# autonomousvision/unimatch

Measured on AMD Instinct MI355X. Metric: image_pairs_per_sec, higher is better.
Workload: dtype f16x2

## Files before the change

include/unimatch_hip.h:

```cpp
#ifndef UNIMATCH_HIP_H
#define UNIMATCH_HIP_H

#include <stddef.h>
#include <stdint.h>

#ifdef __cplusplus
extern "C" {
#endif

#define UM_VERSION 220

#define UM_MODE_EXACT 0
#define UM_MODE_FAST 1

#define UM_ERR_BAD_ARG (-1)
#define UM_ERR_BAD_GEOMETRY (-2)
#define UM_ERR_WORKSPACE (-3)
#define UM_ERR_UNSUPPORTED (-4)
#define UM_ERR_COLLECTIVE (-5)

int um_version(void);
const char* um_last_error_string(void);

#define UM_RANGE_PLANES 1u
// ... 21 lines not shown
#define UM_K_COUNT 12
#define UM_V_WATTN_TILE 0
#define UM_V_WATTN_KSPLIT 1
#define UM_V_FFN_TILE 2
#define UM_V_FFN_HSPLIT 3
#define UM_V_GSV4 4
#define UM_V_GSV3 5
#define UM_V_K4_MFMA 6
#define UM_V_K4_VALU 7
#define UM_V_K3_MFMA 8
#define UM_V_K3_VALU 9
#define UM_V_CONV_PATCH 10
#define UM_V_CONV_ROWS 11
#define UM_V_CONV_GENERIC 12
#define UM_V_WATTN_W8 13
#define UM_V_COUNT 14
int um_census_enable(int on);
long um_census_count(int variant);
int um_window_attn_tile_census(int enable, unsigned long long* counts4);
double um_probe_mfma_flops(int iters);
int um_probe_mfma(float* sink, int iters, void* stream);
int um_probe_copy(const void* src, void* dst, size_t bytes, void* stream);
int um_probe_chase(const unsigned* ring, unsigned* out, int hops, void* stream);
int um_timing_enable(int kernel_mask);
int um_timing_collect(int kernel_id, double* total_ms, int* launches);

size_t um_window_attn_workspace_bytes(int streams, int tokens, int channels, int mode);
int um_window_attn_fwd(const float* q, const float* k, const float* v, float* out,
                       int streams, int h, int w, int channels,
                       int win_h, int win_w, int shift_h, int shift_w,
                       int mode, void* workspace, size_t workspace_bytes, void* stream);
// ... 62 lines not shown

size_t um_stem_planes_bytes(int batch, int h, int w);
size_t um_conv7_planes_bytes(int batch, int h, int w, int stride);
int um_conv7_fwd(const float* image, int channels, int normalize, const float* mean3, const float* std3, void* image_planes,
                 const void* w_planes, const float* bias, float* out, int out_ld, int out_coff, void* out_planes, int outp_ld,
                 int outp_coff, long outp_rows, float* stats_out, int batch, int h, int w, int cout, int stride, int act,
                 int wshift, void* stream);
int um_stem_conv_fwd(const float* image, int normalize, const float* mean3, const float* std3, void* image_planes,
                     const void* w_planes, float* out, float* stats_out, int batch, int h, int w, int cout, int wshift,
                     void* stream);

size_t um_nhwc_norm_workspace_bytes(int batch, int pixels, int channels);
int um_nhwc_instance_norm(const float* x, const float* shortcut, const void* shortcut_planes, void* planes_out, float* f32_out,
                          int batch, int pixels, int channels, float eps, int normalize, int relu, const float* conv_stats,
                          int conv_stats_parts, void* workspace, size_t workspace_bytes, int mode, void* stream);

int um_nhwc_gate(int mode, const float* src, int src_ld, const float* zr, float* hbuf, void* planes_out, int ld, int coff,
                 long plane_rows, long rows, int channels, void* stream);

int um_nchw_to_nhwc(const float* x, void* planes_out, float* f32_out, int batch, int channels, int pixels, int mode,
                    void* stream);

size_t um_global_corr_workspace_bytes(int batch, int tokens, int channels, int mode);
int um_global_corr_softmax_flow(const float* f0, const float* f1, float* flow,
                                int batch, int h, int w, int channels, int bidir,
                                int mode, void* workspace, size_t workspace_bytes, void* stream);

int um_global_corr_softmax_stereo(const float* f0, const float* f1, float* disp,
                                  int batch, int h, int w, int channels,
                                  int mode, void* workspace, size_t workspace_bytes, void* stream);
// ... 96 lines not shown
```

unimatch_amd/_abi.py:

```python
import ctypes
import os

_HERE = os.path.dirname(os.path.abspath(__file__))
LIB_PATH = os.environ.get('UM_LIB') or os.path.join(_HERE, 'libunimatch_hip.so')

MODE_EXACT = 0
MODE_FAST = 1

CENSUS = {'wattn_tile': 0, 'wattn_ksplit': 1, 'ffn_tile': 2, 'ffn_hsplit': 3, 'gsv4': 4, 'gsv3': 5, 'k4_mfma': 6, 'k4_valu': 7,
          'k3_mfma': 8, 'k3_valu': 9, 'conv_patch': 10, 'conv_rows': 11, 'conv_generic': 12, 'wattn_w8': 13}

_c_int, _c_size_t, _c_void_p = ctypes.c_int, ctypes.c_size_t, ctypes.c_void_p

SIGNATURES = {
    'um_version': (_c_int, []),
    'um_last_error_string': (ctypes.c_char_p, []),
    'um_range_flags': (_c_int, [ctypes.POINTER(ctypes.c_uint), _c_int]),
    'um_timing_enable': (_c_int, [_c_int]),
    'um_timing_collect': (_c_int, [_c_int, ctypes.POINTER(ctypes.c_double), ctypes.POINTER(_c_int)]),
    'um_window_attn_workspace_bytes': (_c_size_t, [_c_int] * 4),
    'um_window_attn_fwd': (_c_int, [_c_void_p] * 4 + [_c_int] * 9 + [_c_void_p, _c_size_t, _c_void_p]),
    'um_window_attn_planes_fwd': (_c_int, [_c_void_p] * 4 + [_c_int] * 6 + [ctypes.c_long] * 2 + [_c_int] * 6 + [_c_void_p]),
    'um_window_attn_merge_fwd': (_c_int, [_c_void_p] * 7 + [ctypes.c_float, _c_int, _c_void_p] + [_c_int] * 6 + [ctypes.c_long] * 2 +
                                 [_c_int] * 6 + [_c_void_p]),
    'um_window_attn_qproj_merge_fwd': (_c_int, [_c_void_p] * 8 + [ctypes.c_float, _c_int, _c_void_p] + [_c_int] * 5 + [ctypes.c_long] +
# ... 9 lines not shown
                                _c_void_p]),
    'um_ffn_split_workspace_bytes': (_c_size_t, [_c_int] * 2),
    'um_ffn_kv_fwd': (_c_int, [_c_void_p] * 4 + [_c_int] * 3 + [_c_void_p] * 2 + [ctypes.c_float, _c_void_p, _c_void_p, _c_void_p, _c_int, _c_void_p,
                                _c_size_t, _c_void_p]),
    'um_kv4_fwd': (_c_int, [_c_void_p, _c_void_p, _c_int, _c_int, _c_void_p, _c_int, _c_void_p]),
    'um_conv2d_fwd': (_c_int, [_c_void_p] * 5 + [_c_int] * 13 + [_c_void_p]),
    'um_conv2d_ex': (_c_int, [_c_void_p, _c_int, _c_int, ctypes.c_long, _c_void_p, _c_void_p, _c_void_p, _c_int, _c_int, _c_void_p,
                              _c_int, _c_int, ctypes.c_long, _c_void_p] + [_c_int] * 13 + [_c_void_p]),
    'um_nhwc_gate': (_c_int, [_c_int, _c_void_p, _c_int, _c_void_p, _c_void_p, _c_void_p, _c_int, _c_int, ctypes.c_long, ctypes.c_long,
                              _c_int, _c_void_p]),
    'um_local_corr_with_flow_planes': (_c_int, [_c_void_p] * 4 + [_c_int, ctypes.c_long] + [_c_int] * 5 + [_c_void_p]),
    'um_conv2d_gru_fwd': (_c_int, [_c_int, _c_void_p, _c_int, _c_int, ctypes.c_long, _c_void_p, _c_void_p, _c_void_p, _c_void_p, _c_int,
                                   _c_void_p, _c_int, _c_void_p, _c_int, _c_int, ctypes.c_long] + [_c_int] * 11 + [_c_void_p]),
    'um_conv2d_gru_add_fwd': (_c_int, [_c_int, _c_void_p, _c_int, _c_int, ctypes.c_long, _c_void_p, _c_void_p, _c_void_p, _c_int, _c_void_p, _c_void_p,
                                        _c_int, _c_void_p, _c_int, _c_void_p, _c_int, _c_int, ctypes.c_long] + [_c_int] * 11 + [_c_void_p]),
    'um_conv_stats_bytes': (_c_size_t, [_c_int] * 3),
    'um_conv_stats_parts': (_c_int, [_c_int] * 8),
    'um_stem_planes_bytes': (_c_size_t, [_c_int] * 3),
    'um_conv7_planes_bytes': (_c_size_t, [_c_int] * 4),
    'um_conv7_fwd': (_c_int, [_c_void_p, _c_int, _c_int] + [_c_void_p] * 6 + [_c_int, _c_int, _c_void_p, _c_int, _c_int, ctypes.c_long,
                              _c_void_p] + [_c_int] * 7 + [_c_void_p]),
    'um_stem_conv_fwd': (_c_int, [_c_void_p, _c_int] + [_c_void_p] * 6 + [_c_int] * 5 + [_c_void_p]),
    'um_nhwc_norm_workspace_bytes': (_c_size_t, [_c_int] * 3),
    'um_nhwc_instance_norm': (_c_int, [_c_void_p] * 5 + [_c_int] * 3 + [ctypes.c_float, _c_int, _c_int, _c_void_p, _c_int, _c_void_p,
                                       _c_size_t, _c_int, _c_void_p]),
    'um_nchw_to_nhwc': (_c_int, [_c_void_p] * 3 + [_c_int] * 4 + [_c_void_p]),
    'um_flow_warp': (_c_int, [_c_void_p] * 3 + [_c_int] * 4 + [_c_void_p]),
    'um_fwd_bwd_occlusion': (_c_int, [_c_void_p] * 4 + [_c_int] * 3 + [ctypes.c_float] * 2 + [_c_void_p]),
    'um_flow_to_rgb_workspace_bytes': (_c_size_t, [_c_int] * 3),
    'um_flow_to_rgb': (_c_int, [_c_void_p] * 2 + [_c_int] * 3 + [_c_void_p, _c_size_t, _c_void_p]),
# ... 136 lines not shown
```

unimatch_amd/csrc/conv.hip:

```cpp
#include <cstdlib>
#include <cstring>
#ifndef UM_CONV_2P
#define UM_CONV_2P 0
#endif
#include "common.h"
#include "planes.h"

struct ConvArgs {
    const unsigned short* ap;
    long a_plane_stride;
    unsigned row_stride;
    unsigned zero_row;
    const unsigned short* wp;
    long w_plane_stride;
    const float* bias;
    float* out;
    unsigned short* outp;
    long outp_plane_stride;
    int out_ld, out_coff, outp_ld, outp_coff;
    int act;
    int gate, gate_c, gate_zld;
    float* gate_h;
    const float* gate_z;
    float* gate_hout;
    int gate_hout_ld;
    float* stats;
    const float* addend;
    int addend_ld;
    int B, Hi, Wi, Cin, Ho, Wo, Cout;
    int KH, KW, stride, pad_h, pad_w;
    int M;
    float out_scale;
    int xcd;
};

__device__ __forceinline__ void conv_dma16(const void* base, unsigned byte_off, const unsigned char* lds_dst) {
    const unsigned dst = __builtin_amdgcn_readfirstlane(
        (unsigned)(unsigned long)(const __attribute__((address_space(3))) unsigned char*)lds_dst);
    unsigned keep;
    asm volatile("s_mov_b32 %0, m0\n\ts_mov_b32 m0, %3\n\ts_nop 0\n\tglobal_load_lds_dwordx4 %1, %2\n\ts_mov_b32 m0, %0"
                 : "=&s"(keep)
                 : "v"(byte_off), "s"(base), "s"(dst)
                 : "memory");
}

template <int V>
struct IntC {
    static constexpr int value = V;
// ... 550 lines not shown
template <int NS, int NT>
struct ConvPatchLds {
    static constexpr int NTE = NT < 2 ? NT : 2;
    static constexpr int PW = 34, PPIX = 10 * PW;
    static constexpr int PROWS = 352;
    static constexpr int ATILE = PROWS * 32;
    static constexpr int WTILE = 32 * NT * 32;
    static constexpr int ASLOT = NS * ATILE, WSLOT = NS * 3 * WTILE;
    static constexpr int WBASE = 2 * ASLOT;
    static constexpr int STAGES = 2 * ASLOT + 2 * WSLOT;
    static constexpr int EPI = 8 * 32 * (32 * NTE * 4);
    static constexpr int SCRATCH = 8 * 2 * 32 * NT * 4 + 64;
    static constexpr int TOTAL = (STAGES > EPI + SCRATCH) ? STAGES : EPI + SCRATCH;
};

template <typename T, int NS, int NT>
__global__ __launch_bounds__(512, (NT < 4 ? 2 : 1)) void conv_patch_kernel(ConvArgs a) {
    using L = ConvPatchLds<NS, NT>;
    constexpr int ATILE = L::ATILE, WTILE = L::WTILE, ASLOT = L::ASLOT, WSLOT = L::WSLOT, WBASE = L::WBASE;
    constexpr int PW = L::PW;
    extern __shared__ __attribute__((aligned(16))) unsigned char lds[];

    const int tid = threadIdx.x, lane = tid & 63;
    const int wave = __builtin_amdgcn_readfirstlane(tid >> 6);
    const int half = lane >> 5, fr = lane & 31;
    const int twn = (a.Wo + 31) >> 5, tpi = twn * ((a.Ho + 7) >> 3);
    const int ny = (a.Cout + 32 * NT - 1) / (32 * NT);
    const int wg = a.xcd ? xcd_remap(blockIdx.x, gridDim.x) : blockIdx.x;
    const int tile = wg / ny;
    const int bt = tile / tpi, tt = tile - bt * tpi;
    const int ty = tt / twn, tx = tt - ty * twn;
    const int y0 = ty * 8, x0 = tx * 32;
    const int n0 = (wg - tile * ny) * (32 * NT);
    const int cpt = a.Cin >> 4;
    const int ktot = 9 * a.Cin;

    const int dcp = lane & 1;
    unsigned rowoff[2];
#pragma unroll
    for (int i = 0; i < 2; ++i) {
        const int j = 32 * (wave + 8 * i) + (lane >> 1);
        const int py = j / PW, px = j - py * PW;
        const int iy = y0 - 1 + py, ix = x0 - 1 + px;
        const bool ok = j < L::PPIX && (unsigned)iy < (unsigned)a.Hi && (unsigned)ix < (unsigned)a.Wi;
        const unsigned row = ok ? (unsigned)((bt * a.Hi + iy) * a.Wi + ix) : a.zero_row;
        rowoff[i] = row * a.row_stride;
    }
    auto stage_patch = [&](int cc, unsigned char* buf) {
#pragma unroll
        for (int i = 0; i < 2; ++i)
            if (i == 0 || wave < 3) {
                const int blk = wave + 8 * i;
                const int r = 32 * blk + (lane >> 1);
                const int sc = dcp ^ ((r >> 3) & 1);
                const unsigned off = rowoff[i] + (unsigned)((cc * 16 + 8 * sc) * 2);
#pragma unroll
                for (int pl = 0; pl < NS; ++pl) conv_dma16(a.ap + pl * a.a_plane_stride, off, buf + pl * ATILE + (32 * blk) * 32);
            }
    };
    auto stage_w = [&](int cc, int ky, unsigned char* buf) {
#pragma unroll
        for (int k = 0; k < (3 * NT + 7) / 8; ++k) {
            const int q = wave + 8 * k;
            if (q < 3 * NT) {
                const int kx = q / NT, jb = q - kx * NT;
                const int r = 32 * jb + (lane >> 1);
                const int sc = dcp ^ ((r >> 3) & 1);
                const int n = min(n0 + r, a.Cout - 1);
                const unsigned off = (unsigned)(((long)n * ktot + (ky * 3 + kx) * a.Cin + cc * 16 + 8 * sc) * 2);
#pragma unroll
                for (int pl = 0; pl < NS; ++pl)
                    conv_dma16(a.wp + pl * a.w_plane_stride, off, buf + (kx * NS + pl) * WTILE + (32 * jb) * 32);
            }
// ... 4 lines not shown
#pragma unroll
    for (int nt = 0; nt < NT; ++nt)
#pragma unroll
        for (int r = 0; r < 16; ++r) acc[nt][r] = 0.f;

    const int foffw = fr * 32 + ((half ^ ((fr >> 3) & 1)) << 4);
    int foffa[3][3];
#pragma unroll
    for (int ky = 0; ky < 3; ++ky)
#pragma unroll
        for (int kx = 0; kx < 3; ++kx) {
            const int r = (wave + ky) * PW + kx + fr;
            foffa[ky][kx] = r * 32 + ((half ^ ((r >> 3) & 1)) << 4);
        }

    stage_patch(0, lds);
    stage_w(0, 0, lds + WBASE);
    asm volatile("s_waitcnt vmcnt(0)" ::: "memory");
    __syncthreads();

    for (int cc = 0; cc < cpt; ++cc) {
        const int a_cur = (cc & 1) * ASLOT, a_nxt = ASLOT - a_cur;
#pragma unroll
        for (int ky = 0; ky < 3; ++ky) {
            const int w_par = (cc + ky) & 1;
            const int w_cur = WBASE + w_par * WSLOT, w_nxt = WBASE + (w_par ^ 1) * WSLOT;
            const bool last = ky == 2 && cc + 1 == cpt;
            __builtin_amdgcn_s_setprio(1);
#pragma unroll
            for (int kx = 0; kx < 3; ++kx) {
                if (kx == 0 && !last) stage_w(ky == 2 ? cc + 1 : cc, ky == 2 ? 0 : ky + 1, lds + w_nxt);
                if (kx == 1 && ky == 0 && cc + 1 < cpt) stage_patch(cc + 1, lds + a_nxt);
                const i16x8 bh = *reinterpret_cast<const i16x8*>(lds + a_cur + foffa[ky][kx]);
                i16x8 bl;
                if (NS == 2) bl = *reinterpret_cast<const i16x8*>(lds + a_cur + ATILE + foffa[ky][kx]);
                const unsigned char* wt = lds + w_cur + kx * NS * WTILE;
#pragma unroll
                for (int nt = 0; nt < NT; ++nt) {
                    const i16x8 wh = *reinterpret_cast<const i16x8*>(wt + nt * 32 * 32 + foffw);
                    if (NS == 2) {
                        const i16x8 wl = *reinterpret_cast<const i16x8*>(wt + WTILE + nt * 32 * 32 + foffw);
                        if (UM_CONV_2P != 1) acc[nt] = T::mfma(wl, bh, acc[nt]);
                        if (UM_CONV_2P != 2) acc[nt] = T::mfma(wh, bl, acc[nt]);
                    }
                    acc[nt] = T::mfma(wh, bh, acc[nt]);
                }
            }
            __builtin_amdgcn_s_setprio(0);
            asm volatile("s_waitcnt vmcnt(0)" ::: "memory");
            __syncthreads();
        }
    }
    const int nvalid = y0 + wave < a.Ho ? min(32, a.Wo - x0) : 0;
    conv_epilogue<T, NS, NT, L::NTE>(a, acc, lds, lds + L::EPI, bt, (y0 + wave) * a.Wo + x0, nvalid, (bt * tpi + tt) * 2, true, n0, tid,
                                     wave, lane, half);
}

extern void um_set_error(const char* fmt, ...);

static int conv_xcd_enabled() {
    static const int on = um_debug_env("UM_CONV_NO_XCD") == nullptr;
    return on;
}

template <int NT>
static hipError_t launch_conv(const ConvArgs& a, int mode, hipStream_t stream) {
    dim3 grid(a.B * ((a.Ho * a.Wo + 127) / 128) * ((a.Cout + 32 * NT - 1) / (32 * NT))), block(256);
    ScopedKernelTimer timer(UM_K_CONV, stream);
    um_census_hit(UM_V_CONV_GENERIC);
    if (mode == 0)
// ... 19 lines not shown
            configured[0] = true;
        }
        hipLaunchKernelGGL((conv_rows_kernel<Fp16, 2, NT, KW, NSLOT>), grid, block, LDS2, stream, a);
    } else {
        if (!configured[1]) {
            hipError_t e = hipFuncSetAttribute(reinterpret_cast<const void*>(&conv_rows_kernel<Bf16, 1, NT, KW, NSLOT>),
                                               hipFuncAttributeMaxDynamicSharedMemorySize, LDS1);
            if (e != hipSuccess) return e;
            configured[1] = true;
        }
        hipLaunchKernelGGL((conv_rows_kernel<Bf16, 1, NT, KW, NSLOT>), grid, block, LDS1, stream, a);
    }
    return hipGetLastError();
}

template <int NT>
static hipError_t launch_conv_patch(const ConvArgs& a, int mode, hipStream_t stream) {
    static bool configured[2] = {false, false};
    dim3 grid(a.B * ((a.Ho + 7) / 8) * ((a.Wo + 31) / 32) * ((a.Cout + 32 * NT - 1) / (32 * NT))), block(512);
    constexpr int LDS2 = ConvPatchLds<2, NT>::TOTAL, LDS1 = ConvPatchLds<1, NT>::TOTAL;
    static_assert(LDS2 <= 160 * 1024 && LDS1 <= 160 * 1024, "ring beyond the CU's LDS");
    ScopedKernelTimer timer(UM_K_CONV, stream);
    um_census_hit(UM_V_CONV_PATCH);
    if (mode == 0) {
        if (!configured[0]) {
            hipError_t e = hipFuncSetAttribute(reinterpret_cast<const void*>(&conv_patch_kernel<Fp16, 2, NT>),
                                               hipFuncAttributeMaxDynamicSharedMemorySize, LDS2);
            if (e != hipSuccess) return e;
            configured[0] = true;
        }
        hipLaunchKernelGGL((conv_patch_kernel<Fp16, 2, NT>), grid, block, LDS2, stream, a);
    } else {
        if (!configured[1]) {
            hipError_t e = hipFuncSetAttribute(reinterpret_cast<const void*>(&conv_patch_kernel<Bf16, 1, NT>),
                                               hipFuncAttributeMaxDynamicSharedMemorySize, LDS1);
            if (e != hipSuccess) return e;
            configured[1] = true;
        }
        hipLaunchKernelGGL((conv_patch_kernel<Bf16, 1, NT>), grid, block, LDS1, stream, a);
    }
    return hipGetLastError();
}

enum ConvKind { CONV_GENERIC = 0, CONV_ROWS = 1, CONV_PATCH = 2 };

static ConvKind conv_pick(int hi, int wi, int ho, int wo, int cout, int kh, int kw, int stride, int pad_h, int pad_w, int* nt_out) {
    const int nt = (cout % 128 == 0 || cout > 192) ? 4 : (cout % 96 == 0) ? 3 : (cout <= 64 || cout % 64 == 0) ? 2 : 4;
    *nt_out = nt;
    static const bool rows_enabled = um_debug_env("UM_CONV_NO_ROWS") == nullptr;
    static const char* patch_env = um_debug_env("UM_CONV_PATCH");
    static const char* patch_nts = patch_env ? patch_env : "234";
    const bool same = stride == 1 && ho == hi && wo == wi && (long)ho * wo >= 256 && rows_enabled;
    const bool rows3 = same && kw == 3 && pad_w == 1, rows5 = same && kw == 5 && pad_w == 2 && nt == 4;
    const long tiled = (long)((ho + 7) / 8 * 8) * ((wo + 31) / 32 * 32);
    if (rows3 && kh == 3 && pad_h == 1 && 4L * ho * wo >= 3 * tiled && strchr(patch_nts, '0' + nt) != nullptr) {
        if (cout <= 32) *nt_out = 1;
        return CONV_PATCH;
    }
    return rows3 || rows5 ? CONV_ROWS : CONV_GENERIC;
}

extern "C" int um_conv_stats_parts(int hi, int wi, int cout, int kh, int kw, int stride, int pad_h, int pad_w) {
    if (hi <= 0 || wi <= 0 || cout <= 0 || kh <= 0 || kw <= 0 || stride <= 0 || pad_h < 0 || pad_w < 0) return -1;
    const int ho = (hi + 2 * pad_h - kh) / stride + 1, wo = (wi + 2 * pad_w - kw) / stride + 1;
    if (ho <= 0 || wo <= 0) return -1;
    int nt;
    if (conv_pick(hi, wi, ho, wo, cout, kh, kw, stride, pad_h, pad_w, &nt) == CONV_PATCH) return 2 * ((ho + 7) / 8) * ((wo + 31) / 32);
    return (int)(((long)ho * wo + 127) / 128);
}

static int conv2d_impl(const void* a_planes, int a_ld, int a_coff, long a_rows, const void* w_planes, const float* bias,
                       float* out, int out_ld, int out_coff, void* out_planes, int outp_ld, int outp_coff, long outp_rows,
                       float* stats_out, int batch, int hi, int wi, int cin, int cout, int kh, int kw, int stride,
                       int pad_h, int pad_w, int act, int wshift, int mode, void* stream_, int gate, float* gate_h,
                       const float* gate_z, int gate_zld, const float* addend = nullptr, int addend_ld = 0, float* gate_hout = nullptr,
                       int gate_hout_ld = 0) {
    if (gate_hout && (gate != 2 || gate_hout_ld < cout || gate_hout_ld % 4 != 0 || ((unsigned long)gate_hout & 15) != 0)) {
        um_set_error("um_conv2d: a separate new-state tensor goes with gate 2 only: 16-byte aligned fp32 [M][ld >= channels, ld %% 4 == 0]");
        return -1;
    }
    if (addend && (addend_ld < cout || addend_ld % 4 != 0 || ((unsigned long)addend & 15) != 0 || stats_out)) {
        um_set_error("um_conv2d: the addend must be 16-byte aligned fp32 [M][ld >= cout, ld %% 4 == 0] (and excludes fused statistics)");
        return -1;
    }
    if (!a_planes || !w_planes || (!out && !out_planes) || batch <= 0 || hi <= 0 || wi <= 0 || cin <= 0 || cin % 32 != 0 ||
        cout <= 0 || cout % 4 != 0 || kh <= 0 || kw <= 0 || stride <= 0 || pad_h < 0 || pad_w < 0 || (mode != 0 && mode != 1) ||
        wshift < 0 || wshift > 14 || act < 0 || act > 3) {
        um_set_error("um_conv2d: bad argument (batch=%d hi=%d wi=%d cin=%d cout=%d k=%dx%d stride=%d pad=%d,%d act=%d; cin must "
                     "be a multiple of 32, cout of 4)", batch, hi, wi, cin, cout, kh, kw, stride, pad_h, pad_w, act);
        return -1;
    }
    const int ho = (hi + 2 * pad_h - kh) / stride + 1, wo = (wi + 2 * pad_w - kw) / stride + 1;
    if (ho <= 0 || wo <= 0) {
        um_set_error("um_conv2d: empty output (%d x %d)", ho, wo);
        return -1;
    }
    const long rows_in = (long)batch * hi * wi, m = (long)batch * ho * wo;
    if (a_ld < a_coff + cin || a_ld % 8 != 0 || a_coff % 8 != 0 || a_rows < rows_in + 1 ||
        (out && (out_ld < out_coff + cout || out_ld % 4 != 0 || out_coff % 4 != 0)) ||
        (out_planes && (outp_ld < outp_coff + (gate == 1 ? cout / 2 : cout) || outp_ld % 4 != 0 || outp_coff % 4 != 0 ||
// ... 1 lines not shown
        um_set_error("um_conv2d: inconsistent leading dimensions / offsets / row counts");
        return -1;
    }
    if (stats_out && !out) {
        um_set_error("um_conv2d: fused statistics need the fp32 output");
        return -1;
    }
    if (bias && ((unsigned long)bias & 15) != 0) {
        um_set_error("um_conv2d: bias must be 16-byte aligned");
        return -1;
    }
    if (a_rows * a_ld * 2 >= (1L << 32) || (long)cout * kh * kw * cin * 2 >= (1L << 32) || m >= (1L << 31)) {
        um_set_error("um_conv2d: operand planes beyond 4 GiB are not addressable by this kernel");
        return -4;
    }
    ConvArgs a;
    a.ap = (const unsigned short*)a_planes + a_coff;
    a.a_plane_stride = a_rows * a_ld;
    a.row_stride = (unsigned)a_ld * 2;
    a.zero_row = (unsigned)(a_rows - 1);
    a.wp = (const unsigned short*)w_planes;
    a.w_plane_stride = (long)cout * kh * kw * cin;
    a.bias = bias;
    a.out = out;
    a.out_ld = out_ld;
    a.out_coff = out_coff;
    a.outp = (unsigned short*)out_planes;
    a.outp_ld = outp_ld;
    a.outp_coff = outp_coff;
    a.outp_plane_stride = outp_rows * outp_ld;
    a.stats = stats_out;
// ... 14 lines not shown
    a.M = (int)m;
    a.act = act;
    a.gate = gate;
    a.gate_c = gate == 1 ? cout / 2 : cout;
    a.gate_h = gate_h;
    a.gate_z = gate_z;
    a.gate_zld = gate_zld;
    a.gate_hout = gate_hout ? gate_hout : gate_h;
    a.gate_hout_ld = gate_hout ? gate_hout_ld : a.gate_c;
    a.out_scale = ldexpf(1.f, -wshift);
    a.xcd = conv_xcd_enabled();
    hipError_t e;
    int nt;
    const ConvKind kind = conv_pick(hi, wi, ho, wo, cout, kh, kw, stride, pad_h, pad_w, &nt);
    hipStream_t st = (hipStream_t)stream_;
    if (kind == CONV_PATCH)
        e = nt == 1 ? launch_conv_patch<1>(a, mode, st) : nt == 2 ? launch_conv_patch<2>(a, mode, st) : nt == 3 ? launch_conv_patch<3>(a, mode, st)
                                                                                                          : launch_conv_patch<4>(a, mode, st);
    else if (kind == CONV_ROWS && kw == 5) e = launch_conv_rows<4, 5, 2>(a, mode, st);
    else if (kind == CONV_ROWS) e = nt == 2 ? launch_conv_rows<2, 3, 2>(a, mode, st) : nt == 3 ? launch_conv_rows<3, 3, 2>(a, mode, st) : launch_conv_rows<4, 3, 2>(a, mode, st);
    else e = nt == 2 ? launch_conv<2>(a, mode, st) : nt == 3 ? launch_conv<3>(a, mode, st) : launch_conv<4>(a, mode, st);
    if (e != hipSuccess) {
        um_set_error("um_conv2d: launch failed: %s", hipGetErrorString(e));
        return (int)e;
    }
    return 0;
}

extern "C" int um_conv2d_ex(const void* a_planes, int a_ld, int a_coff, long a_rows, const void* w_planes, const float* bias,
                            float* out, int out_ld, int out_coff, void* out_planes, int outp_ld, int outp_coff, long outp_rows,
                            float* stats_out, int batch, int hi, int wi, int cin, int cout, int kh, int kw, int stride,
// ... 33 lines not shown
    if (gate == 1)
        return conv2d_impl(a_planes, a_ld, a_coff, a_rows, w_planes, bias, z_out, z_out_ld, 0, out_planes, outp_ld, outp_coff,
                           outp_rows, nullptr, batch, hi, wi, cin, 2 * channels, kh, kw, 1, pad_h, pad_w, 2, wshift, mode, stream_,
                           1, hidden, nullptr, 0, addend, addend_ld);
    return conv2d_impl(a_planes, a_ld, a_coff, a_rows, w_planes, bias, nullptr, 0, 0, out_planes, outp_ld, outp_coff, outp_rows,
                       nullptr, batch, hi, wi, cin, channels, kh, kw, 1, pad_h, pad_w, 3, wshift, mode, stream_, 2, hidden, z, z_ld,
                       addend, addend_ld, z_out, z_out_ld);
}

extern "C" int um_conv2d_fwd(const void* a_planes, const void* w_planes, const float* bias, float* out, float* stats_out,
                             int batch, int hi, int wi, int cin, int cout, int kh, int kw, int stride, int pad_h, int pad_w,
                             int relu, int wshift, int mode, void* stream_) {
    const long rows_in = (long)batch * hi * wi;
    return um_conv2d_ex(a_planes, cin, 0, rows_in + 1, w_planes, bias, out, cout, 0, nullptr, 0, 0, 0, stats_out, batch, hi, wi,
                        cin, cout, kh, kw, stride, pad_h, pad_w, relu ? 1 : 0, wshift, mode, stream_);
}

template <int CPP>
__global__ __launch_bounds__(256) void pack7_kernel(const float* img, unsigned short* planes, long plane_stride, int B, int C,
                                                    int H, int W, int Hp, int Wp, int normalize, float m0, float m1, float m2,
                                                    float s0, float s1, float s2) {
    const long idx = (long)blockIdx.x * 256 + threadIdx.x;
    const long total = (long)B * Hp * Wp;
    if (idx >= total) return;
    const int xp = (int)(idx % Wp);
    const long t = idx / Wp;
    const int yp = (int)(t % Hp), b = (int)(t / Hp);
    const int y = yp - 3, x = xp - 3;
    float v[CPP];
#pragma unroll
// ... 98 lines not shown
    a.Wo = wo;
    a.Cout = cout;
    a.KH = 7;
    a.KW = 1;
    a.stride = stride;
    a.pad_h = 0;
    a.pad_w = 0;
    a.M = (int)m;
    a.act = act;
    a.gate = 0;
    a.gate_c = a.gate_zld = 0;
    a.gate_h = nullptr;
    a.gate_z = nullptr;
    a.out_scale = ldexpf(1.f, -wshift);
    a.xcd = conv_xcd_enabled();
    hipError_t e;
    if (cout % 128 == 0 || cout > 192) e = launch_conv<4>(a, 0, stream);
    else if (cout % 96 == 0) e = launch_conv<3>(a, 0, stream);
    else e = launch_conv<2>(a, 0, stream);
    if (e != hipSuccess) {
        um_set_error("um_conv7_fwd: launch failed: %s", hipGetErrorString(e));
        return (int)e;
    }
    return 0;
}

extern "C" size_t um_stem_planes_bytes(int batch, int h, int w) { return um_conv7_planes_bytes(batch, h, w, 2); }

extern "C" int um_stem_conv_fwd(const float* image, int normalize, const float* mean3, const float* std3, void* image_planes,
                                const void* w_planes, float* out, float* stats_out, int batch, int h, int w, int cout,
// ... 5 lines not shown
```

unimatch_amd/csrc/nhwc_ops.hip:

```cpp
#include "common.h"
#include "planes.h"

#define NHWC_CHUNK_ROWS 256

__global__ __launch_bounds__(256) void nhwc_stats_kernel(const float* x, float* partial, int P, int C, int nchunk) {
    __shared__ float red[2][256 * 4];
    const int b = blockIdx.y, ch = blockIdx.x;
    const int quads = C >> 2, rl_n = 256 / quads;
    const int q = threadIdx.x % quads, rl = threadIdx.x / quads;
    const int r0 = ch * NHWC_CHUNK_ROWS, r1 = min(P, r0 + NHWC_CHUNK_ROWS);
    const float* xb = x + ((long)b * P) * C + 4 * q;
    f32x4 s1 = {0.f, 0.f, 0.f, 0.f}, s2 = s1;
    if (rl < rl_n) {
        const f32x4 k = *reinterpret_cast<const f32x4*>(xb + (long)r0 * C);
        for (int r = r0 + rl; r < r1; r += rl_n) {
            const f32x4 v = *reinterpret_cast<const f32x4*>(xb + (long)r * C) - k;
            s1 += v;
            s2 += v * v;
        }
    }
#pragma unroll
    for (int i = 0; i < 4; ++i) {
        red[0][threadIdx.x * 4 + i] = s1[i];
        red[1][threadIdx.x * 4 + i] = s2[i];
// ... 315 lines not shown
    const dim3 grid((unsigned)((total + 255) / 256));
    if (mode == 0)
        hipLaunchKernelGGL((nhwc_apply_kernel<Fp16, 2>), grid, dim3(256), 0, stream, x, stats, shortcut,
                           (const unsigned short*)shortcut_planes, (unsigned short*)planes_out, f32_out, rows, pixels, channels, relu);
    else
        hipLaunchKernelGGL((nhwc_apply_kernel<Bf16, 1>), grid, dim3(256), 0, stream, x, stats, shortcut,
                           (const unsigned short*)shortcut_planes, (unsigned short*)planes_out, f32_out, rows, pixels, channels, relu);
    const hipError_t e = hipGetLastError();
    if (e != hipSuccess) {
        um_set_error("um_nhwc_instance_norm: launch failed: %s", hipGetErrorString(e));
        return (int)e;
    }
    return 0;
}

extern "C" int um_nchw_to_nhwc(const float* x, void* planes_out, float* f32_out, int batch, int channels, int pixels, int mode,
                               void* stream_) {
    hipStream_t stream = (hipStream_t)stream_;
    if (!x || (!planes_out && !f32_out) || batch <= 0 || pixels <= 0 || channels <= 0 || channels % 8 != 0 || channels > 256 ||
        (mode != 0 && mode != 1)) {
        um_set_error("um_nchw_to_nhwc: bad argument (batch=%d channels=%d pixels=%d: channels must be a multiple of 8, <= 256)",
                     batch, channels, pixels);
        return -1;
    }
    const long rows = (long)batch * pixels;
    const dim3 grid((pixels + 63) / 64, batch);
    ScopedKernelTimer timer(UM_K_INSTANCE_NORM, stream);
    if (mode == 0)
        hipLaunchKernelGGL((nchw_to_nhwc_kernel<Fp16, 2>), grid, dim3(256), 0, stream, x, (unsigned short*)planes_out, f32_out,
                           pixels, channels, rows);
// ... 33 lines not shown
```

unimatch_amd/encoder.py:

```python

import torch
import torch.nn as nn
import torch.nn.functional as F


def _conv3(cin, cout, stride=1):
    return nn.Conv2d(cin, cout, 3, stride=stride, padding=1, bias=False)


class _Residual(nn.Module):

    def __init__(self, cin, cout, stride):
        super().__init__()
        self.conv1, self.conv2 = _conv3(cin, cout, stride), _conv3(cout, cout)
        self.norm1, self.norm2 = nn.InstanceNorm2d(cout), nn.InstanceNorm2d(cout)
        self.downsample = None
        if stride != 1 or cin != cout:
            self.norm3 = nn.InstanceNorm2d(cout)
            self.downsample = nn.Sequential(nn.Conv2d(cin, cout, 1, stride=stride), self.norm3)

    def forward(self, x, ops=None):
        if ops is not None:
            y = ops.instance_norm(self.conv1(x), relu=True)
            sc = x if self.downsample is None else ops.instance_norm(self.downsample[0](x), relu=False)
            return ops.instance_norm(self.conv2(y), relu=True, shortcut=sc.contiguous())
        y = F.relu(self.norm1(self.conv1(x)))
        y = F.relu(self.norm2(self.conv2(y)))
        return F.relu((x if self.downsample is None else self.downsample(x)) + y)


    def forward_nhwc(self, act, ops, want_f32):
        planes, f32, b, h, w, c = act
        stride = self.conv1.stride[0]
        cout = self.conv1.out_channels
        t, ho, wo = ops.conv2d_nhwc((planes, b, h, w, c), self.conv1.weight, None, stride, (1, 1), stats=True)
        tp, _ = ops.nhwc_norm(t, b, ho * wo, relu=True, want_planes=True, conv_stats=ops.last_conv_stats)
        u, _, _ = ops.conv2d_nhwc((tp, b, ho, wo, cout), self.conv2.weight, None, 1, (1, 1), stats=True)
        ustats = ops.last_conv_stats
        sc = scp = None
        if self.downsample is None:
            sc, scp = (f32, None) if f32 is not None else (None, planes)
        else:
            proj = self.downsample[0]
            d, _, _ = ops.conv2d_nhwc((planes, b, h, w, c), proj.weight, proj.bias, stride, (0, 0), stats=True)
            _, sc = ops.nhwc_norm(d, b, ho * wo, relu=False, want_planes=False, want_f32=True, conv_stats=ops.last_conv_stats)
        op, of = ops.nhwc_norm(u, b, ho * wo, relu=True, shortcut=sc, shortcut_planes=scp, want_planes=True, want_f32=want_f32,
                               conv_stats=ustats)
        return op, of, b, ho, wo, cout


class _SharedStridedConv(nn.Module):

# ... 78 lines not shown
```

unimatch_amd/ops.py:

```python
import contextlib
import ctypes
import threading
import weakref
from collections import namedtuple

import torch

from . import _abi

PRECISIONS = {'exact': _abi.MODE_EXACT, 'fast': _abi.MODE_FAST}


class KernelTimer:

    def __init__(self):
        self.records = []

    def summary(self):
        torch.cuda.synchronize()
        out = {}
        for name, s, e, meta in self.records:
            d = out.setdefault(name, {'calls': 0, 'ms': 0.0, 'meta': meta})
            d['calls'] += 1
            d['ms'] += s.elapsed_time(e)
# ... 89 lines not shown
    def release_cached_planes(self):
        for k in [k for k in self._entries if isinstance(k.kind, tuple)]:
            del self._entries[k]


class HipOps(WorkspaceRegistry):

    fused_tail = True
    fused_ffn = True
    fused_merge = True
    fused_qproj = True
    block_kv = True
    refine_hoist = True
    fused_kv = True
    fused_conv = True
    CONV_MODE = 0
    WSHIFT = 10

    def __init__(self, precision='exact'):
        if precision not in PRECISIONS:
            raise ValueError(f'precision must be one of {sorted(PRECISIONS)}')
        self.lib = _abi.load()
        if not torch.cuda.is_available():
            raise _abi.HipExtensionError('no GPU visible: the UniMatch hot path only runs on the HIP extension')
        self.precision = precision
        self.mode = PRECISIONS[precision]
        self.timer = None
        self.nplanes = 2 if precision == 'exact' else 1
        self._wcache = {}
        self.cache_generation = 0
# ... 354 lines not shown
        ho, wo = (h + 2 * ph - kh) // stride + 1, (w + 2 * pw - kw) // stride + 1
        out = torch.empty((b * ho * wo, cout), dtype=torch.float32, device=planes.device)
        self.last_conv_stats = None
        if stats:
            parts = self.lib.um_conv_stats_parts(h, w, cout, kh, kw, stride, ph, pw)
            self.last_conv_stats = (torch.empty(self.lib.um_conv_stats_bytes(b, parts, cout) // 4, dtype=torch.float32,
                                                device=planes.device), parts)
        st = self.last_conv_stats[0] if self.last_conv_stats is not None else None
        meta = {'flops': 2.0 * b * ho * wo * cout * kh * kw * cin}
        code = self._launch('conv', lambda: self.lib.um_conv2d_fwd(
            _ptr(planes), _ptr(wp), _ptr(bias) if bias is not None else None, _ptr(out), _ptr(st) if st is not None else None,
            b, h, w, cin, cout, kh, kw,
            stride, ph, pw, int(bool(relu)), self.WSHIFT, self.CONV_MODE, _stream()), meta)
        _abi.check(code, 'um_conv2d_fwd')
        return out, ho, wo

    def nhwc_planes_from(self, pieces, pad_to=32):
        rows = pieces[0].shape[0]
        c = sum(p.shape[1] for p in pieces)
        cp = (c + pad_to - 1) // pad_to * pad_to
        if cp != c:
            pieces = list(pieces) + [torch.zeros((rows, cp - c), dtype=torch.float32, device=pieces[0].device)]
        x = pieces[0].contiguous() if len(pieces) == 1 else torch.cat(list(pieces), 1)
        planes, _ = self.nhwc_norm(x, 1, rows, normalize=False, relu=False, want_planes=True)
        return planes, cp

    def conv_weight_padded(self, weight, cin_to):
        key, hit = self._cache_get(('padw', cin_to), (weight,))
        if hit is None:
            cout, cin, kh, kw = weight.shape
# ... 365 lines not shown
```

Measured before the change: 875.9.

## Apply instance norm and ReLU on load inside the patch conv kernel

```diff
diff --git a/include/unimatch_hip.h b/include/unimatch_hip.h
--- a/include/unimatch_hip.h
+++ b/include/unimatch_hip.h
@@ -59,7 +59,8 @@
 #define UM_V_CONV_ROWS 11
 #define UM_V_CONV_GENERIC 12
 #define UM_V_WATTN_W8 13
-#define UM_V_COUNT 14
+#define UM_V_CONV_PATCH_NORM 14
+#define UM_V_COUNT 15
 int um_census_enable(int on);
 long um_census_count(int variant);
 int um_window_attn_tile_census(int enable, unsigned long long* counts4);
@@ -152,6 +153,13 @@
 int um_nhwc_instance_norm(const float* x, const float* shortcut, const void* shortcut_planes, void* planes_out, float* f32_out,
                           int batch, int pixels, int channels, float eps, int normalize, int relu, const float* conv_stats,
                           int conv_stats_parts, void* workspace, size_t workspace_bytes, int mode, void* stream);
+
+int um_nhwc_stats_finalize(const float* conv_stats, int conv_stats_parts, float* stats_out, int batch, int pixels, int channels,
+                           float eps, void* stream);
+int um_conv2d_norm_supported(int hi, int wi, int cin, int cout, int kh, int kw, int stride, int pad_h, int pad_w, int mode);
+int um_conv2d_norm_fwd(const float* x, const float* norm_stats, int norm_relu, const void* w_planes, const float* bias, float* out,
+                       float* stats_out, int batch, int hi, int wi, int cin, int cout, int kh, int kw, int stride, int pad_h,
+                       int pad_w, int relu, int wshift, int mode, void* stream);
 
 int um_nhwc_gate(int mode, const float* src, int src_ld, const float* zr, float* hbuf, void* planes_out, int ld, int coff,
                  long plane_rows, long rows, int channels, void* stream);
diff --git a/unimatch_amd/_abi.py b/unimatch_amd/_abi.py
--- a/unimatch_amd/_abi.py
+++ b/unimatch_amd/_abi.py
@@ -8,7 +8,7 @@
 MODE_FAST = 1
 
 CENSUS = {'wattn_tile': 0, 'wattn_ksplit': 1, 'ffn_tile': 2, 'ffn_hsplit': 3, 'gsv4': 4, 'gsv3': 5, 'k4_mfma': 6, 'k4_valu': 7,
-          'k3_mfma': 8, 'k3_valu': 9, 'conv_patch': 10, 'conv_rows': 11, 'conv_generic': 12, 'wattn_w8': 13}
+          'k3_mfma': 8, 'k3_valu': 9, 'conv_patch': 10, 'conv_rows': 11, 'conv_generic': 12, 'wattn_w8': 13, 'conv_patch_norm': 14}
 
 _c_int, _c_size_t, _c_void_p = ctypes.c_int, ctypes.c_size_t, ctypes.c_void_p
 
@@ -48,6 +48,9 @@
                                    _c_void_p, _c_int, _c_void_p, _c_int, _c_int, ctypes.c_long] + [_c_int] * 11 + [_c_void_p]),
     'um_conv2d_gru_add_fwd': (_c_int, [_c_int, _c_void_p, _c_int, _c_int, ctypes.c_long, _c_void_p, _c_void_p, _c_void_p, _c_int, _c_void_p, _c_void_p,
                                         _c_int, _c_void_p, _c_int, _c_void_p, _c_int, _c_int, ctypes.c_long] + [_c_int] * 11 + [_c_void_p]),
+    'um_conv2d_norm_supported': (_c_int, [_c_int] * 10),
+    'um_conv2d_norm_fwd': (_c_int, [_c_void_p, _c_void_p, _c_int] + [_c_void_p] * 4 + [_c_int] * 13 + [_c_void_p]),
+    'um_nhwc_stats_finalize': (_c_int, [_c_void_p, _c_int, _c_void_p] + [_c_int] * 3 + [ctypes.c_float, _c_void_p]),
     'um_conv_stats_bytes': (_c_size_t, [_c_int] * 3),
     'um_conv_stats_parts': (_c_int, [_c_int] * 8),
     'um_stem_planes_bytes': (_c_size_t, [_c_int] * 3),
diff --git a/unimatch_amd/csrc/conv.hip b/unimatch_amd/csrc/conv.hip
--- a/unimatch_amd/csrc/conv.hip
+++ b/unimatch_amd/csrc/conv.hip
@@ -32,6 +32,9 @@
     int M;
     float out_scale;
     int xcd;
+    const float* xf;
+    const float* nstats;
+    int norm_relu;
 };
 
 __device__ __forceinline__ void conv_dma16(const void* base, unsigned byte_off, const unsigned char* lds_dst) {
@@ -612,12 +615,13 @@
     static constexpr int TOTAL = (STAGES > EPI + SCRATCH) ? STAGES : EPI + SCRATCH;
 };
 
-template <typename T, int NS, int NT>
-__global__ __launch_bounds__(512, (NT < 4 ? 2 : 1)) void conv_patch_kernel(ConvArgs a) {
+typedef const __attribute__((address_space(4))) float* um_const_f32p;
+
+template <typename T, int NS, int NT, bool NORM>
+__device__ __forceinline__ void conv_patch_body(const ConvArgs& a, unsigned char* lds) {
     using L = ConvPatchLds<NS, NT>;
     constexpr int ATILE = L::ATILE, WTILE = L::WTILE, ASLOT = L::ASLOT, WSLOT = L::WSLOT, WBASE = L::WBASE;
     constexpr int PW = L::PW;
-    extern __shared__ __attribute__((aligned(16))) unsigned char lds[];
 
     const int tid = threadIdx.x, lane = tid & 63;
     const int wave = __builtin_amdgcn_readfirstlane(tid >> 6);
@@ -641,8 +645,12 @@
         const int py = j / PW, px = j - py * PW;
         const int iy = y0 - 1 + py, ix = x0 - 1 + px;
         const bool ok = j < L::PPIX && (unsigned)iy < (unsigned)a.Hi && (unsigned)ix < (unsigned)a.Wi;
-        const unsigned row = ok ? (unsigned)((bt * a.Hi + iy) * a.Wi + ix) : a.zero_row;
-        rowoff[i] = row * a.row_stride;
+        if constexpr (NORM) {
+            rowoff[i] = ok ? (unsigned)((bt * a.Hi + iy) * a.Wi + ix) * (unsigned)(a.Cin * 4) : ~0u;
+        } else {
+            const unsigned row = ok ? (unsigned)((bt * a.Hi + iy) * a.Wi + ix) : a.zero_row;
+            rowoff[i] = row * a.row_stride;
+        }
     }
     auto stage_patch = [&](int cc, unsigned char* buf) {
 #pragma unroll
@@ -655,6 +663,43 @@
 #pragma unroll
                 for (int pl = 0; pl < NS; ++pl) conv_dma16(a.ap + pl * a.a_plane_stride, off, buf + pl * ATILE + (32 * blk) * 32);
             }
+    };
+    const int nsc = dcp ^ ((lane >> 4) & 1);
+    f32x4 nx0, nx1;
+    auto norm_load = [&](int cc, int i) {
+        const unsigned off = (rowoff[i] == ~0u ? 0u : rowoff[i]) + (unsigned)((cc * 16 + 8 * nsc) * 4);
+        const unsigned char* p = reinterpret_cast<const unsigned char*>(a.xf) + off;
+        nx0 = *reinterpret_cast<const f32x4*>(p);
+        nx1 = *reinterpret_cast<const f32x4*>(p + 16);
+    };
+    auto norm_store = [&](int cc, int i, unsigned char* buf) {
+        const um_const_f32p mu = (um_const_f32p)(unsigned long)(a.nstats + ((long)bt * 2) * a.Cin + cc * 16);
+        const um_const_f32p rs = mu + a.Cin;
+        float v[8];
+#pragma unroll
+        for (int k = 0; k < 8; ++k) {
+            const float m = nsc ? mu[8 + k] : mu[k], r = nsc ? rs[8 + k] : rs[k];
+            v[k] = ((k < 4 ? nx0[k & 3] : nx1[k & 3]) - m) * r;
+        }
+        if (a.norm_relu) {
+#pragma unroll
+            for (int k = 0; k < 8; ++k) v[k] = fmaxf(v[k], 0.f);
+        }
+        const bool ok = rowoff[i] != ~0u;
+        u32x4 h = {T::pack2(v[0], v[1]), T::pack2(v[2], v[3]), T::pack2(v[4], v[5]), T::pack2(v[6], v[7])};
+        unsigned char* dst = buf + (32 * (wave + 8 * i)) * 32 + lane * 16;
+        if (NS == 2) {
+            u32x4 l;
+#pragma unroll
+            for (int k = 0; k < 4; ++k) {
+                const f32x2 u = T::unpack2(h[k]);
+                l[k] = ok ? T::pack2(v[2 * k] - u[0], v[2 * k + 1] - u[1]) : 0u;
+            }
+            *reinterpret_cast<u32x4*>(dst + ATILE) = l;
+        }
+#pragma unroll
+        for (int k = 0; k < 4; ++k) h[k] = ok ? h[k] : 0u;
+        *reinterpret_cast<u32x4*>(dst) = h;
     };
     auto stage_w = [&](int cc, int ky, unsigned char* buf) {
 #pragma unroll
@@ -689,8 +734,18 @@
             foffa[ky][kx] = r * 32 + ((half ^ ((r >> 3) & 1)) << 4);
         }
 
-    stage_patch(0, lds);
-    stage_w(0, 0, lds + WBASE);
+    if constexpr (NORM) {
+        stage_w(0, 0, lds + WBASE);
+        norm_load(0, 0);
+        norm_store(0, 0, lds);
+        if (wave < 3) {
+            norm_load(0, 1);
+            norm_store(0, 1, lds);
+        }
+    } else {
+        stage_patch(0, lds);
+        stage_w(0, 0, lds + WBASE);
+    }
     asm volatile("s_waitcnt vmcnt(0)" ::: "memory");
     __syncthreads();
 
@@ -705,7 +760,18 @@
 #pragma unroll
             for (int kx = 0; kx < 3; ++kx) {
                 if (kx == 0 && !last) stage_w(ky == 2 ? cc + 1 : cc, ky == 2 ? 0 : ky + 1, lds + w_nxt);
-                if (kx == 1 && ky == 0 && cc + 1 < cpt) stage_patch(cc + 1, lds + a_nxt);
+                if constexpr (NORM) {
+                    if (kx == 1 && cc + 1 < cpt) {
+                        if (ky == 0) norm_load(cc + 1, 0);
+                        if (ky == 1) {
+                            norm_store(cc + 1, 0, lds + a_nxt);
+                            if (wave < 3) norm_load(cc + 1, 1);
+                        }
+                        if (ky == 2 && wave < 3) norm_store(cc + 1, 1, lds + a_nxt);
+                    }
+                } else {
+                    if (kx == 1 && ky == 0 && cc + 1 < cpt) stage_patch(cc + 1, lds + a_nxt);
+                }
                 const i16x8 bh = *reinterpret_cast<const i16x8*>(lds + a_cur + foffa[ky][kx]);
                 i16x8 bl;
                 if (NS == 2) bl = *reinterpret_cast<const i16x8*>(lds + a_cur + ATILE + foffa[ky][kx]);
@@ -729,6 +795,18 @@
     const int nvalid = y0 + wave < a.Ho ? min(32, a.Wo - x0) : 0;
     conv_epilogue<T, NS, NT, L::NTE>(a, acc, lds, lds + L::EPI, bt, (y0 + wave) * a.Wo + x0, nvalid, (bt * tpi + tt) * 2, true, n0, tid,
                                      wave, lane, half);
+}
+
+template <typename T, int NS, int NT>
+__global__ __launch_bounds__(512, (NT < 4 ? 2 : 1)) void conv_patch_kernel(ConvArgs a) {
+    extern __shared__ __attribute__((aligned(16))) unsigned char lds[];
+    conv_patch_body<T, NS, NT, false>(a, lds);
+}
+
+template <typename T, int NS, int NT>
+__global__ __launch_bounds__(512, (NT < 4 ? 2 : 1)) void conv_patch_norm_kernel(ConvArgs a) {
+    extern __shared__ __attribute__((aligned(16))) unsigned char lds[];
+    conv_patch_body<T, NS, NT, true>(a, lds);
 }
 
 extern void um_set_error(const char* fmt, ...);
@@ -778,7 +856,7 @@
     return hipGetLastError();
 }
 
-template <int NT>
+template <int NT, bool NORM = false>
 static hipError_t launch_conv_patch(const ConvArgs& a, int mode, hipStream_t stream) {
     static bool configured[2] = {false, false};
     dim3 grid(a.B * ((a.Ho + 7) / 8) * ((a.Wo + 31) / 32) * ((a.Cout + 32 * NT - 1) / (32 * NT))), block(512);
@@ -786,22 +864,29 @@
     static_assert(LDS2 <= 160 * 1024 && LDS1 <= 160 * 1024, "ring beyond the CU's LDS");
     ScopedKernelTimer timer(UM_K_CONV, stream);
     um_census_hit(UM_V_CONV_PATCH);
+    if (NORM) um_census_hit(UM_V_CONV_PATCH_NORM);
+    void (*k2)(ConvArgs), (*k1)(ConvArgs);
+    if constexpr (NORM) {
+        k2 = conv_patch_norm_kernel<Fp16, 2, NT>;
+        k1 = conv_patch_norm_kernel<Bf16, 1, NT>;
+    } else {
+        k2 = conv_patch_kernel<Fp16, 2, NT>;
+        k1 = conv_patch_kernel<Bf16, 1, NT>;
+    }
     if (mode == 0) {
         if (!configured[0]) {
-            hipError_t e = hipFuncSetAttribute(reinterpret_cast<const void*>(&conv_patch_kernel<Fp16, 2, NT>),
-                                               hipFuncAttributeMaxDynamicSharedMemorySize, LDS2);
+            hipError_t e = hipFuncSetAttribute(reinterpret_cast<const void*>(k2), hipFuncAttributeMaxDynamicSharedMemorySize, LDS2);
             if (e != hipSuccess) return e;
             configured[0] = true;
         }
-        hipLaunchKernelGGL((conv_patch_kernel<Fp16, 2, NT>), grid, block, LDS2, stream, a);
+        hipLaunchKernelGGL(k2, grid, block, LDS2, stream, a);
     } else {
         if (!configured[1]) {
-            hipError_t e = hipFuncSetAttribute(reinterpret_cast<const void*>(&conv_patch_kernel<Bf16, 1, NT>),
-                                               hipFuncAttributeMaxDynamicSharedMemorySize, LDS1);
+            hipError_t e = hipFuncSetAttribute(reinterpret_cast<const void*>(k1), hipFuncAttributeMaxDynamicSharedMemorySize, LDS1);
             if (e != hipSuccess) return e;
             configured[1] = true;
         }
-        hipLaunchKernelGGL((conv_patch_kernel<Bf16, 1, NT>), grid, block, LDS1, stream, a);
+        hipLaunchKernelGGL(k1, grid, block, LDS1, stream, a);
     }
     return hipGetLastError();
 }
@@ -824,6 +909,19 @@
     return rows3 || rows5 ? CONV_ROWS : CONV_GENERIC;
 }
 
+static constexpr bool kNormOnLoad[5] = {false, false, true, true, true};
+
+extern "C" int um_conv2d_norm_supported(int hi, int wi, int cin, int cout, int kh, int kw, int stride, int pad_h, int pad_w, int mode) {
+    if (hi <= 0 || wi <= 0 || cin <= 0 || cin % 32 != 0 || cout <= 0 || cout % 4 != 0 || kh <= 0 || kw <= 0 || stride <= 0 || pad_h < 0 ||
+        pad_w < 0 || (mode != 0 && mode != 1))
+        return 0;
+    const int ho = (hi + 2 * pad_h - kh) / stride + 1, wo = (wi + 2 * pad_w - kw) / stride + 1;
+    if (ho <= 0 || wo <= 0) return 0;
+    int nt;
+    if (conv_pick(hi, wi, ho, wo, cout, kh, kw, stride, pad_h, pad_w, &nt) != CONV_PATCH) return 0;
+    return nt >= 2 && nt <= 4 && kNormOnLoad[nt] ? 1 : 0;
+}
+
 extern "C" int um_conv_stats_parts(int hi, int wi, int cout, int kh, int kw, int stride, int pad_h, int pad_w) {
     if (hi <= 0 || wi <= 0 || cout <= 0 || kh <= 0 || kw <= 0 || stride <= 0 || pad_h < 0 || pad_w < 0) return -1;
     const int ho = (hi + 2 * pad_h - kh) / stride + 1, wo = (wi + 2 * pad_w - kw) / stride + 1;
@@ -838,7 +936,8 @@
                        float* stats_out, int batch, int hi, int wi, int cin, int cout, int kh, int kw, int stride,
                        int pad_h, int pad_w, int act, int wshift, int mode, void* stream_, int gate, float* gate_h,
                        const float* gate_z, int gate_zld, const float* addend = nullptr, int addend_ld = 0, float* gate_hout = nullptr,
-                       int gate_hout_ld = 0) {
+                       int gate_hout_ld = 0, const float* norm_x = nullptr, const float* norm_stats = nullptr, int norm_relu = 0) {
+    const bool norm = norm_x != nullptr;
     if (gate_hout && (gate != 2 || gate_hout_ld < cout || gate_hout_ld % 4 != 0 || ((unsigned long)gate_hout & 15) != 0)) {
         um_set_error("um_conv2d: a separate new-state tensor goes with gate 2 only: 16-byte aligned fp32 [M][ld >= channels, ld %% 4 == 0]");
         return -1;
@@ -847,7 +946,7 @@
         um_set_error("um_conv2d: the addend must be 16-byte aligned fp32 [M][ld >= cout, ld %% 4 == 0] (and excludes fused statistics)");
         return -1;
     }
-    if (!a_planes || !w_planes || (!out && !out_planes) || batch <= 0 || hi <= 0 || wi <= 0 || cin <= 0 || cin % 32 != 0 ||
+    if ((!a_planes && !norm) || !w_planes || (!out && !out_planes) || batch <= 0 || hi <= 0 || wi <= 0 || cin <= 0 || cin % 32 != 0 ||
         cout <= 0 || cout % 4 != 0 || kh <= 0 || kw <= 0 || stride <= 0 || pad_h < 0 || pad_w < 0 || (mode != 0 && mode != 1) ||
         wshift < 0 || wshift > 14 || act < 0 || act > 3) {
         um_set_error("um_conv2d: bad argument (batch=%d hi=%d wi=%d cin=%d cout=%d k=%dx%d stride=%d pad=%d,%d act=%d; cin must "
@@ -879,7 +978,25 @@
         um_set_error("um_conv2d: operand planes beyond 4 GiB are not addressable by this kernel");
         return -4;
     }
+    if (norm) {
+        if (!norm_stats || ((unsigned long)norm_x & 15) != 0 || ((unsigned long)norm_stats & 3) != 0) {
+            um_set_error("um_conv2d_norm_fwd: the fp32 input must be 16-byte aligned and comes with its statistics [batch][2][cin]");
+            return -1;
+        }
+        if (!um_conv2d_norm_supported(hi, wi, cin, cout, kh, kw, stride, pad_h, pad_w, mode)) {
+            um_set_error("um_conv2d_norm_fwd: no on-load kernel for this geometry (hi=%d wi=%d cin=%d cout=%d k=%dx%d stride=%d pad=%d,%d): "
+                         "ask um_conv2d_norm_supported() first", hi, wi, cin, cout, kh, kw, stride, pad_h, pad_w);
+            return -2;
+        }
+        if (rows_in * cin * 4 >= (1L << 32) - 1) {
+            um_set_error("um_conv2d_norm_fwd: an fp32 input beyond 4 GiB is not addressable by this kernel");
+            return -4;
+        }
+    }
     ConvArgs a;
+    a.xf = norm_x;
+    a.nstats = norm_stats;
+    a.norm_relu = norm_relu;
     a.ap = (const unsigned short*)a_planes + a_coff;
     a.a_plane_stride = a_rows * a_ld;
     a.row_stride = (unsigned)a_ld * 2;
@@ -924,7 +1041,9 @@
     int nt;
     const ConvKind kind = conv_pick(hi, wi, ho, wo, cout, kh, kw, stride, pad_h, pad_w, &nt);
     hipStream_t st = (hipStream_t)stream_;
-    if (kind == CONV_PATCH)
+    if (norm)
+        e = nt == 2 ? launch_conv_patch<2, true>(a, mode, st) : nt == 3 ? launch_conv_patch<3, true>(a, mode, st) : launch_conv_patch<4, true>(a, mode, st);
+    else if (kind == CONV_PATCH)
         e = nt == 1 ? launch_conv_patch<1>(a, mode, st) : nt == 2 ? launch_conv_patch<2>(a, mode, st) : nt == 3 ? launch_conv_patch<3>(a, mode, st)
                                                                                                           : launch_conv_patch<4>(a, mode, st);
     else if (kind == CONV_ROWS && kw == 5) e = launch_conv_rows<4, 5, 2>(a, mode, st);
@@ -988,6 +1107,19 @@
     const long rows_in = (long)batch * hi * wi;
     return um_conv2d_ex(a_planes, cin, 0, rows_in + 1, w_planes, bias, out, cout, 0, nullptr, 0, 0, 0, stats_out, batch, hi, wi,
                         cin, cout, kh, kw, stride, pad_h, pad_w, relu ? 1 : 0, wshift, mode, stream_);
+}
+
+extern "C" int um_conv2d_norm_fwd(const float* x, const float* norm_stats, int norm_relu, const void* w_planes, const float* bias, float* out,
+                                  float* stats_out, int batch, int hi, int wi, int cin, int cout, int kh, int kw, int stride, int pad_h,
+                                  int pad_w, int relu, int wshift, int mode, void* stream_) {
+    if (!x) {
+        um_set_error("um_conv2d_norm_fwd: no input");
+        return -1;
+    }
+    const long rows_in = (long)batch * hi * wi;
+    return conv2d_impl(nullptr, cin, 0, rows_in + 1, w_planes, bias, out, cout, 0, nullptr, 0, 0, 0, stats_out, batch, hi, wi, cin, cout, kh,
+                       kw, stride, pad_h, pad_w, relu ? 1 : 0, wshift, mode, stream_, 0, nullptr, nullptr, 0, nullptr, 0, nullptr, 0, x,
+                       norm_stats, norm_relu ? 1 : 0);
 }
 
 template <int CPP>
@@ -1116,6 +1248,8 @@
     a.gate_z = nullptr;
     a.out_scale = ldexpf(1.f, -wshift);
     a.xcd = conv_xcd_enabled();
+    a.xf = a.nstats = nullptr;
+    a.norm_relu = 0;
     hipError_t e;
     if (cout % 128 == 0 || cout > 192) e = launch_conv<4>(a, 0, stream);
     else if (cout % 96 == 0) e = launch_conv<3>(a, 0, stream);
diff --git a/unimatch_amd/csrc/nhwc_ops.hip b/unimatch_amd/csrc/nhwc_ops.hip
--- a/unimatch_amd/csrc/nhwc_ops.hip
+++ b/unimatch_amd/csrc/nhwc_ops.hip
@@ -353,6 +353,25 @@
     return 0;
 }
 
+extern "C" int um_nhwc_stats_finalize(const float* conv_stats, int conv_stats_parts, float* stats_out, int batch, int pixels, int channels,
+                                      float eps, void* stream_) {
+    hipStream_t stream = (hipStream_t)stream_;
+    if (!conv_stats || conv_stats_parts <= 0 || !stats_out || batch <= 0 || pixels <= 0 || !nhwc_channels_ok(channels)) {
+        um_set_error("um_nhwc_stats_finalize: bad argument (parts=%d batch=%d pixels=%d channels=%d: channels must be a multiple of 8, "
+                     "<= 256)", conv_stats_parts, batch, pixels, channels);
+        return -1;
+    }
+    ScopedKernelTimer timer(UM_K_INSTANCE_NORM, stream);
+    hipLaunchKernelGGL(nhwc_stats_finalize_kernel, dim3(channels / 8, batch), dim3(256), 0, stream, conv_stats, stats_out, pixels, channels,
+                       conv_stats_parts, 0, eps);
+    const hipError_t e = hipGetLastError();
+    if (e != hipSuccess) {
+        um_set_error("um_nhwc_stats_finalize: launch failed: %s", hipGetErrorString(e));
+        return (int)e;
+    }
+    return 0;
+}
+
 extern "C" int um_nchw_to_nhwc(const float* x, void* planes_out, float* f32_out, int batch, int channels, int pixels, int mode,
                                void* stream_) {
     hipStream_t stream = (hipStream_t)stream_;
diff --git a/unimatch_amd/encoder.py b/unimatch_amd/encoder.py
--- a/unimatch_amd/encoder.py
+++ b/unimatch_amd/encoder.py
@@ -34,8 +34,11 @@
         stride = self.conv1.stride[0]
         cout = self.conv1.out_channels
         t, ho, wo = ops.conv2d_nhwc((planes, b, h, w, c), self.conv1.weight, None, stride, (1, 1), stats=True)
-        tp, _ = ops.nhwc_norm(t, b, ho * wo, relu=True, want_planes=True, conv_stats=ops.last_conv_stats)
-        u, _, _ = ops.conv2d_nhwc((tp, b, ho, wo, cout), self.conv2.weight, None, 1, (1, 1), stats=True)
+        if getattr(ops, 'norm_on_load', False) and ops.conv2d_norm_supported(ho, wo, cout, self.conv2.weight):
+            u, _, _ = ops.conv2d_nhwc_normed(t, ops.last_conv_stats, (b, ho, wo, cout), self.conv2.weight, stats=True)
+        else:
+            tp, _ = ops.nhwc_norm(t, b, ho * wo, relu=True, want_planes=True, conv_stats=ops.last_conv_stats)
+            u, _, _ = ops.conv2d_nhwc((tp, b, ho, wo, cout), self.conv2.weight, None, 1, (1, 1), stats=True)
         ustats = ops.last_conv_stats
         sc = scp = None
         if self.downsample is None:
diff --git a/unimatch_amd/ops.py b/unimatch_amd/ops.py
--- a/unimatch_amd/ops.py
+++ b/unimatch_amd/ops.py
@@ -127,6 +127,7 @@
     refine_hoist = True
     fused_kv = True
     fused_conv = True
+    norm_on_load = True
     CONV_MODE = 0
     WSHIFT = 10
 
@@ -511,6 +512,37 @@
             stride, ph, pw, int(bool(relu)), self.WSHIFT, self.CONV_MODE, _stream()), meta)
         _abi.check(code, 'um_conv2d_fwd')
         return out, ho, wo
+
+    def conv2d_norm_supported(self, h, w, cin, weight, stride=1, padding=(1, 1)):
+        cout, wcin, kh, kw = weight.shape
+        ph, pw = (padding, padding) if isinstance(padding, int) else padding
+        return wcin == cin and bool(self.lib.um_conv2d_norm_supported(h, w, cin, cout, kh, kw, stride, ph, pw, self.CONV_MODE))
+
+    def conv2d_nhwc_normed(self, x, conv_stats, geom, weight, bias=None, norm_relu=True, relu=False, stats=False, eps=1e-5):
+        b, h, w, cin = geom
+        self._check_rows('x', x, cin)
+        if x.shape[0] != b * h * w:
+            raise ValueError('conv2d_nhwc_normed: x must have b * h * w rows')
+        wp, cout, wcin, kh, kw = self.conv_weight_planes(weight)
+        if wcin != cin:
+            raise ValueError(f'conv2d_nhwc_normed: weight expects {wcin} input channels, activation has {cin}')
+        nstats = torch.empty((b, 2, cin), dtype=torch.float32, device=x.device)
+        _abi.check(self._launch('instance_norm', lambda: self.lib.um_nhwc_stats_finalize(
+            _ptr(conv_stats[0]), conv_stats[1], _ptr(nstats), b, h * w, cin, float(eps), _stream())), 'um_nhwc_stats_finalize')
+        out = torch.empty((b * h * w, cout), dtype=torch.float32, device=x.device)
+        self.last_conv_stats = None
+        if stats:
+            parts = self.lib.um_conv_stats_parts(h, w, cout, kh, kw, 1, 1, 1)
+            self.last_conv_stats = (torch.empty(self.lib.um_conv_stats_bytes(b, parts, cout) // 4, dtype=torch.float32,
+                                                device=x.device), parts)
+        st = self.last_conv_stats[0] if self.last_conv_stats is not None else None
+        meta = {'flops': 2.0 * b * h * w * cout * kh * kw * cin}
+        code = self._launch('conv', lambda: self.lib.um_conv2d_norm_fwd(
+            _ptr(x), _ptr(nstats), int(bool(norm_relu)), _ptr(wp), _ptr(bias) if bias is not None else None, _ptr(out),
+            _ptr(st) if st is not None else None, b, h, w, cin, cout, kh, kw, 1, 1, 1, int(bool(relu)), self.WSHIFT, self.CONV_MODE,
+            _stream()), meta)
+        _abi.check(code, 'um_conv2d_norm_fwd')
+        return out, h, w
 
     def nhwc_planes_from(self, pieces, pad_to=32):
         rows = pieces[0].shape[0]
```

After: 904.5, median of 6. +3.3%, better.
